# svenstaro/bvh

Measured on NVIDIA H100. Metric: traversal_Mrays_per_s, higher is better.
Workload: dtype f32

## Files before the change

bvh_b200/csrc/traverse.cu:

```cuda
#include "internal.h"
#include "csr.cuh"
#include "queries.cuh"
#include <cstdlib>
#include <cstring>
#include <algorithm>
#include <chrono>

namespace bvhb200 {

static inline uint32_t pick_slots(bvhgpu_ctx* ctx, uint32_t nrays) {
    if (ctx->traverse_slots >= 0) return (uint32_t)std::min<int64_t>(ctx->traverse_slots, 64);
    uint64_t budget_words = 1ull << 30;
    if (ctx->slot_budget_words == 0) {
        size_t free_b = 0, total_b = 0;
        ctx->slot_budget_words = cudaMemGetInfo(&free_b, &total_b) == cudaSuccess ? std::max<uint64_t>((uint64_t)free_b / 16, 1) : budget_words;
    }
    budget_words = std::min<uint64_t>(budget_words, ctx->slot_budget_words);
    const uint64_t k = budget_words / std::max<uint32_t>(nrays, 1u);
    if (k < 4) return (uint32_t)k;
    uint32_t p = 4;
    while (p * 2 <= k && p < 64) p *= 2;
    return p;
}

template <class T> static inline const typename Traits<T>::DAabb* walk_aabbs(const Tree<T>* tree) { return tree->dims == 2 && tree->d_aabb_trav ? tree->d_aabb_trav : tree->d_aabb; }

constexpr int SCAN_ITEMS = 8;
constexpr int SCAN_THREADS = 256;
constexpr int SCAN_TILE = SCAN_ITEMS * SCAN_THREADS;
static_assert(SCAN_THREADS == CSR_SCAN_THREADS && SCAN_TILE == CSR_SCAN_TILE, "scan geometry declared in internal.h");

template <class T> __device__ __forceinline__ T tmin2(T a, T b);
template <> __device__ __forceinline__ float tmin2(float a, float b) { return fminf(a, b); }
template <> __device__ __forceinline__ double tmin2(double a, double b) { return fmin(a, b); }
template <class T> __device__ __forceinline__ T tmax2(T a, T b);
template <> __device__ __forceinline__ float tmax2(float a, float b) { return fmaxf(a, b); }
template <> __device__ __forceinline__ double tmax2(double a, double b) { return fmax(a, b); }

template <class T>
__device__ __forceinline__ bool slab_hit(const T o[3], const T inv[3], const T mn[3], const T mx[3]) {
    const T l0 = mul_rn(sub_rn(mn[0], o[0]), inv[0]), r0 = mul_rn(sub_rn(mx[0], o[0]), inv[0]);
    const T l1 = mul_rn(sub_rn(mn[1], o[1]), inv[1]), r1 = mul_rn(sub_rn(mx[1], o[1]), inv[1]);
    const T l2 = mul_rn(sub_rn(mn[2], o[2]), inv[2]), r2 = mul_rn(sub_rn(mx[2], o[2]), inv[2]);
    const bool nan = (l0 != l0) | (r0 != r0) | (l1 != l1) | (r1 != r1) | (l2 != l2) | (r2 != r2);
    const T tmin = tmax2(tmax2(tmin2(l0, r0), tmin2(l1, r1)), tmin2(l2, r2));
    const T tmax = tmin2(tmin2(tmax2(l0, r0), tmax2(l1, r1)), tmax2(l2, r2));
    const T lo = tmin > T(0) ? tmin : T(0);
    return !nan && tmax >= lo;
}

template <class T, bool FLAT, class Emit>
__device__ __forceinline__ uint32_t walk(const typename Traits<T>::TNode* __restrict__ trec, uint32_t n_rec,
                                         const typename Traits<T>::DAabb* __restrict__ aabb,
                                         const T o[3], const T inv[3], Emit emit) {
    uint32_t i = 0, visits = 0;
    while (i < n_rec) {
        T mn[3], mx[3];
        uint32_t skip, shape;
        fetch(trec + i, mn, mx, skip, shape);
        ++visits;
        if (slab_hit(o, inv, mn, mx)) {
            if (shape != BVH_INVALID) {
                bool report = true;
                if (FLAT) {
                    T smn[3], smx[3];
                    load_aabb(aabb + shape, smn, smx);
                    report = slab_hit(o, inv, smn, smx);
                }
                if (report) emit(shape);
            }
            i = i + 1;
        } else {
            i = skip;
        }
    }
    return visits;
}

template <class T> struct RaySrc { const T* base; uint32_t fmt; };
constexpr uint32_t RAYS_FULL = 0, RAYS_OD = 1;
template <class T, bool L2>
__device__ __forceinline__ void load_ray(const RaySrc<T>& src, size_t r, T o[3], T inv[3]) {
    if (src.fmt == RAYS_FULL) {
        const T* p = src.base + 9 * r;
#pragma unroll
        for (int k = 0; k < 3; ++k) { o[k] = L2 ? __ldcg(p + k) : __ldg(p + k); inv[k] = L2 ? __ldcg(p + 6 + k) : __ldg(p + 6 + k); }
    } else {
        const T* p = src.base + 6 * r;
#pragma unroll
        for (int k = 0; k < 3; ++k) { o[k] = L2 ? __ldcg(p + k) : __ldg(p + k); inv[k] = div_rn(T(1), L2 ? __ldcg(p + 3 + k) : __ldg(p + 3 + k)); }
    }
}

template <class T>
__global__ void __launch_bounds__(256) coherence_probe_kernel(RaySrc<T> rays, uint32_t nrays, uint32_t* flag) {
    __shared__ float acc[8];
    float sum = 0.f;
    const uint32_t samples = 1024, stride = nrays > 2 * samples ? nrays / samples : 1;
    const uint32_t rstride = rays.fmt == RAYS_FULL ? 9u : 6u;
    uint32_t n = 0;
    for (uint32_t k = threadIdx.x; k < samples; k += 256) {
        const uint32_t i = k * stride;
        if (i + 1 >= nrays) break;
        const T* a = rays.base + (size_t)rstride * i + 3;
        const T* b = rays.base + (size_t)rstride * (i + 1) + 3;
        sum += (float)(a[0] * b[0] + a[1] * b[1] + a[2] * b[2]);
        ++n;
    }
    for (int o = 16; o > 0; o >>= 1) { sum += __shfl_xor_sync(0xffffffffu, sum, o); n += __shfl_xor_sync(0xffffffffu, n, o); }
    __shared__ uint32_t cnt[8];
    if (lane_id() == 0) { acc[threadIdx.x >> 5] = sum; cnt[threadIdx.x >> 5] = n; }
    __syncthreads();
    if (threadIdx.x == 0) {
        float s = 0.f; uint32_t c = 0;
        for (int w = 0; w < 8; ++w) { s += acc[w]; c += cnt[w]; }
        *flag = (c > 0 && s / (float)c > 0.9f) ? 1u : 0u;
    }
}

template <class T, bool FLAT>
__global__ void __launch_bounds__(256) walk_count_kernel(const typename Traits<T>::TNode* __restrict__ trec, uint32_t n_rec,
                                                         const typename Traits<T>::DAabb* __restrict__ aabb,
                                                         RaySrc<T> rays, uint32_t nrays,
                                                         uint32_t first, uint32_t count,
                                                         uint32_t* __restrict__ counts, uint32_t* __restrict__ slots, uint32_t K,
                                                         unsigned long long* __restrict__ visit_total, const uint32_t* __restrict__ gate, uint32_t run_if) {
    if (gate && *gate != run_if) return;
    const uint32_t r = first + blockIdx.x * blockDim.x + threadIdx.x;
    uint32_t visits = 0;
    if (r < first + count) {
        T o[3], inv[3];
        load_ray<T, false>(rays, r, o, inv);
        uint32_t cnt = 0;
        visits = walk<T, FLAT>(trec, n_rec, aabb, o, inv, [&](uint32_t shape) {
            if (cnt < K) slots[(size_t)cnt * nrays + r] = shape;
            ++cnt;
        });
        counts[r] = cnt;
    }
    visits = __reduce_add_sync(0xffffffffu, visits);
    if (lane_id() == 0 && visits) atomicAdd(visit_total, (unsigned long long)visits);
}

template <class T, bool FLAT, bool STREAM>
__global__ void __launch_bounds__(256) walk_persistent_kernel(const typename Traits<T>::TNode* __restrict__ trec, uint32_t n_rec,
                                                              const typename Traits<T>::DAabb* __restrict__ aabb,
                                                              RaySrc<T> rays, uint32_t nrays,
                                                              uint32_t* __restrict__ ticket, const uint32_t* ready,
                                                              uint32_t* __restrict__ counts, uint32_t* __restrict__ slots, uint32_t K,
                                                              unsigned long long* __restrict__ visit_total, const uint32_t* __restrict__ gate, uint32_t run_if,
                                                              uint32_t* err, unsigned long long timeout_ns) {
    if (gate && *gate != run_if) return;
    constexpr uint32_t NONE = 0xFFFFFFFFu;
    constexpr int REFILL = 8;
    const uint32_t FULL = 0xffffffffu;
    const uint32_t lane = lane_id(), lt = lanemask_lt();
    uint32_t r = NONE, i = 0, cnt = 0, visits = 0;
    bool loaded = false;
    T o[3] = {T(0), T(0), T(0)}, inv[3] = {T(0), T(0), T(0)};
    bool exhausted = false;
    for (;;) {
        const uint32_t need = __ballot_sync(FULL, r == NONE);
        if (need && !exhausted) {
            uint32_t base = 0;
            if (lane == 0) base = atomicAdd(ticket, (uint32_t)__popc(need));
            base = __shfl_sync(FULL, base, 0);
            if (base >= nrays) exhausted = true;
            const uint32_t mine = base + __popc(need & lt);
            if (r == NONE && mine < nrays) {
                r = mine; i = 0; cnt = 0;
                if (STREAM) loaded = false;
                else load_ray<T, false>(rays, mine, o, inv);
            }
        }
        if (STREAM) {
            const uint32_t pend = __ballot_sync(FULL, r != NONE && !loaded);
            if (pend) {
                const bool any_active = __ballot_sync(FULL, r != NONE && loaded) != 0u;
                const uint32_t lowest = __reduce_min_sync(FULL, (r != NONE && !loaded) ? r : NONE);
                uint32_t rd = 0, ok = 1;
                if (lane == 0) {
                    rd = *(volatile const uint32_t*)ready;
                    if (!any_active && rd <= lowest) {
                        uint32_t ns = 100;
                        const unsigned long long t0 = global_timer_ns();
                        while (rd <= lowest) {
                            if (*(volatile const uint32_t*)err != 0u) { ok = 0; break; }
                            if (global_timer_ns() - t0 > timeout_ns) { ok = 0; atomicExch(err, (uint32_t)BVHGPU_ERR_TIMEOUT); break; }
                            __nanosleep(ns);
                            if (ns < 2000) ns <<= 1;
                            rd = *(volatile const uint32_t*)ready;
                        }
                    }
                }
                rd = __shfl_sync(FULL, rd, 0);
                ok = __shfl_sync(FULL, ok, 0);
                if (!ok) {
                    exhausted = true;
                    if (r != NONE && !loaded) r = NONE;
                } else if (__ballot_sync(FULL, r != NONE && !loaded && r < rd)) {
                    __threadfence();
                    if (r != NONE && !loaded && r < rd) { load_ray<T, true>(rays, r, o, inv); loaded = true; }
                }
            }
        }
        if (__ballot_sync(FULL, r != NONE) == 0) break;
        uint32_t rounds = 0;
        for (;;) {
            if (r != NONE && (!STREAM || loaded)) {
                T mn[3], mx[3];
                uint32_t skip, shape;
                fetch(trec + i, mn, mx, skip, shape);
                ++visits;
                if (slab_hit(o, inv, mn, mx)) {
                    if (shape != BVH_INVALID) {
                        bool report = true;
                        if (FLAT) {
                            T smn[3], smx[3];
                            load_aabb(aabb + shape, smn, smx);
                            report = slab_hit(o, inv, smn, smx);
                        }
                        if (report) { if (cnt < K) slots[(size_t)cnt * nrays + r] = shape; ++cnt; }
                    }
                    i = i + 1;
                } else {
                    i = skip;
                }
                if (i >= n_rec) { counts[r] = cnt; r = NONE; }
            }
            const uint32_t idle_mask = __ballot_sync(FULL, r == NONE);
            const int idle = __popc(idle_mask);
            if (idle == 32 || (idle >= REFILL && !exhausted)) break;
            if (STREAM) {
                const uint32_t pend = __ballot_sync(FULL, r != NONE && !loaded);
                if (pend && (((++rounds) & 15u) == 0u || (pend | idle_mask) == FULL)) break;
            }
        }
    }
    visits = __reduce_add_sync(FULL, visits);
    if (lane == 0 && visits) atomicAdd(visit_total, (unsigned long long)visits);
}

template <bool FLAT, bool STREAM, int VPC>
__global__ void __launch_bounds__(1024, 1) walk_top_kernel(const TNodeF* __restrict__ trec, const DAabbF* __restrict__ aabb,
                                                           uint32_t n_rec, const float4* __restrict__ top,
                                                           RaySrc<float> rays, uint32_t nrays, uint32_t* __restrict__ ticket, const uint32_t* ready,
                                                           uint32_t* __restrict__ counts, uint32_t* __restrict__ slots, uint32_t K,
                                                           unsigned long long* __restrict__ visit_total, const uint32_t* __restrict__ gate, uint32_t run_if,
                                                           uint32_t* err, unsigned long long timeout_ns, int refill) {
    extern __shared__ float4 s_top[];
    if (gate && *gate != run_if) return;
    const uint32_t n_top = reinterpret_cast<const uint32_t*>(top)[0];
    for (uint32_t k = threadIdx.x; k < 2 * n_top; k += blockDim.x) s_top[k] = top[2 + k];
    __syncthreads();
    uint32_t s_lo;
    asm volatile("mov.u32 %0, %1;" : "=r"(s_lo) : "r"((uint32_t)__cvta_generic_to_shared(s_top)));
    const uint32_t s_hi = s_lo + 16u * n_top;
    constexpr uint32_t NONE = 0xFFFFFFFFu;
    const uint32_t FULL = 0xffffffffu;
    const uint32_t lane = lane_id(), lt = lanemask_lt();
    uint32_t r = NONE, j = 0, g = 0, gend = 0, cnt = 0, visits = 0;
    bool loaded = false;
    float o[3] = {0.f, 0.f, 0.f}, inv[3] = {0.f, 0.f, 0.f};
    bool exhausted = false;
    for (;;) {
        const uint32_t need = __ballot_sync(FULL, r == NONE);
        if (need && !exhausted) {
            uint32_t base = 0;
            if (lane == 0) base = atomicAdd(ticket, (uint32_t)__popc(need));
            base = __shfl_sync(FULL, base, 0);
            if (base >= nrays) exhausted = true;
            const uint32_t mine = base + __popc(need & lt);
            if (r == NONE && mine < nrays) {
                r = mine; j = 0; cnt = 0; g = 0; gend = n_top ? 0u : n_rec;
                if (STREAM) loaded = false;
                else load_ray<float, false>(rays, mine, o, inv);
            }
        }
        if (STREAM) {
            const uint32_t pend = __ballot_sync(FULL, r != NONE && !loaded);
            if (pend) {
                const bool any_active = __ballot_sync(FULL, r != NONE && loaded) != 0u;
                const uint32_t lowest = __reduce_min_sync(FULL, (r != NONE && !loaded) ? r : NONE);
                uint32_t rd = 0, ok = 1;
                if (lane == 0) {
                    rd = *(volatile const uint32_t*)ready;
                    if (!any_active && rd <= lowest) {
                        uint32_t ns = 100;
                        const unsigned long long t0 = global_timer_ns();
                        while (rd <= lowest) {
                            if (*(volatile const uint32_t*)err != 0u) { ok = 0; break; }
                            if (global_timer_ns() - t0 > timeout_ns) { ok = 0; atomicExch(err, (uint32_t)BVHGPU_ERR_TIMEOUT); break; }
                            __nanosleep(ns);
                            if (ns < 2000) ns <<= 1;
                            rd = *(volatile const uint32_t*)ready;
                        }
                    }
                }
                rd = __shfl_sync(FULL, rd, 0);
                ok = __shfl_sync(FULL, ok, 0);
                if (!ok) {
                    exhausted = true;
                    if (r != NONE && !loaded) r = NONE;
                } else if (__ballot_sync(FULL, r != NONE && !loaded && r < rd)) {
                    __threadfence();
                    if (r != NONE && !loaded && r < rd) { load_ray<float, true>(rays, r, o, inv); loaded = true; }
                }
            }
        }
        if (__ballot_sync(FULL, r != NONE) == 0) break;
        const int leave = exhausted ? 32 : refill;
        auto visit = [&]() {
            if (r != NONE && (!STREAM || loaded)) {
                float mn[3], mx[3];
                uint32_t w3, w7;
                const bool below = g < gend;
                if (!below) {
                    float4 a, b;
                    asm("ld.shared.v4.f32 {%0,%1,%2,%3}, [%4];" : "=f"(a.x), "=f"(a.y), "=f"(a.z), "=f"(a.w) : "r"(s_lo + 16u * j));
                    asm("ld.shared.v4.f32 {%0,%1,%2,%3}, [%4];" : "=f"(b.x), "=f"(b.y), "=f"(b.z), "=f"(b.w) : "r"(s_hi + 16u * j));
                    mn[0] = a.x; mn[1] = a.y; mn[2] = a.z; w3 = __float_as_uint(a.w);
                    mx[0] = b.x; mx[1] = b.y; mx[2] = b.z; w7 = __float_as_uint(b.w);
                } else {
                    fetch(trec + g, mn, mx, w3, w7);
                }
                ++visits;
                const bool hit = slab_hit(o, inv, mn, mx);
                const bool fringe = !below && (w7 + 0x80000000u) < 0x7FFFFFFFu;
                const uint32_t cur = below ? g : j;
                const uint32_t nxt = (hit || fringe) ? cur + 1 : w3;
                if (hit && (int32_t)w7 >= 0) {
                    bool report = true;
                    if (FLAT) {
                        float smn[3], smx[3];
                        load_aabb(aabb + w7, smn, smx);
                        report = slab_hit(o, inv, smn, smx);
                    }
                    if (report) { if (cnt < K) slots[(size_t)cnt * nrays + r] = w7; ++cnt; }
                }
                j = below ? j : nxt;
                gend = below ? gend : ((hit && fringe) ? w3 : 0u);
                g = below ? nxt : (w7 & 0x7FFFFFFFu);
                if (g >= gend && j >= n_top) { counts[r] = cnt; r = NONE; }
            }
        };
        uint32_t rounds = 0;
        for (;;) {
#pragma unroll
            for (int u = 0; u < VPC; ++u) visit();
            const uint32_t idle_mask = __ballot_sync(FULL, r == NONE);
            if (__popc(idle_mask) >= leave) break;
            if (STREAM) {
                const uint32_t pend = __ballot_sync(FULL, r != NONE && !loaded);
                if (pend && (((rounds += VPC) & 15u) == 0u || (pend | idle_mask) == FULL)) break;
            }
        }
    }
    visits = __reduce_add_sync(FULL, visits);
    if (lane == 0 && visits) atomicAdd(visit_total, (unsigned long long)visits);
}

__global__ void __launch_bounds__(SCAN_THREADS) scan_local_kernel(const uint32_t* __restrict__ counts, uint32_t n,
                                                                  uint32_t* __restrict__ local, unsigned long long* __restrict__ blocksum,
                                                                  uint32_t* __restrict__ maxcount) {
    __shared__ uint32_t wsum[SCAN_THREADS / 32];
    const uint32_t base = blockIdx.x * SCAN_TILE + threadIdx.x * SCAN_ITEMS;
    uint32_t v[SCAN_ITEMS], s = 0, m = 0;
#pragma unroll
    for (int k = 0; k < SCAN_ITEMS; ++k) { v[k] = (base + k < n) ? counts[base + k] : 0u; s += v[k]; m = v[k] > m ? v[k] : m; }
    uint32_t incl = s;
#pragma unroll
    for (int o = 1; o < 32; o <<= 1) { const uint32_t t = __shfl_up_sync(0xffffffffu, incl, o); if ((int)lane_id() >= o) incl += t; }
    if (lane_id() == 31) wsum[threadIdx.x >> 5] = incl;
    if (maxcount) { m = __reduce_max_sync(0xffffffffu, m); if (lane_id() == 0 && m) atomicMax(maxcount, m); }
    __syncthreads();
    uint32_t woff = 0;
    for (int w = 0; w < (int)(threadIdx.x >> 5); ++w) woff += wsum[w];
    uint32_t run = woff + incl - s;
#pragma unroll
    for (int k = 0; k < SCAN_ITEMS; ++k) { if (base + k < n) local[base + k] = run; run += v[k]; }
    if (threadIdx.x == SCAN_THREADS - 1) blocksum[blockIdx.x] = (unsigned long long)(woff + incl);
}
__global__ void __launch_bounds__(1024) scan_blocks_kernel(unsigned long long* __restrict__ blocksum, uint32_t nblocks,
                                                           unsigned long long* __restrict__ total) {
    __shared__ unsigned long long wsum[32];
    __shared__ unsigned long long carry_s;
    if (threadIdx.x == 0) carry_s = *total;
    __syncthreads();
    for (uint32_t b0 = 0; b0 < nblocks; b0 += 1024) {
        const uint32_t b = b0 + threadIdx.x;
        const unsigned long long v = b < nblocks ? blocksum[b] : 0ull;
        unsigned long long incl = v;
#pragma unroll
        for (int o = 1; o < 32; o <<= 1) { const unsigned long long t = __shfl_up_sync(0xffffffffu, incl, o); if ((int)lane_id() >= o) incl += t; }
        if (lane_id() == 31) wsum[threadIdx.x >> 5] = incl;
        __syncthreads();
        unsigned long long woff = 0;
        for (int w = 0; w < (int)(threadIdx.x >> 5); ++w) woff += wsum[w];
        const unsigned long long carry = carry_s;
        if (b < nblocks) blocksum[b] = carry + woff + incl - v;
        __syncthreads();
        if (threadIdx.x == 1023) carry_s = carry + woff + incl;
        __syncthreads();
    }
    if (threadIdx.x == 0) *total = carry_s;
}

__device__ __forceinline__ void st_release_sys(unsigned long long* p, unsigned long long v) {
    asm volatile("st.release.sys.global.u64 [%0], %1;" ::"l"(p), "l"(v) : "memory");
}
__device__ __forceinline__ unsigned long long ld_acquire_sys(const unsigned long long* p) {
    unsigned long long v;
    asm volatile("ld.acquire.sys.global.u64 %0, [%1];" : "=l"(v) : "l"(p) : "memory");
    return v;
}
constexpr int MB_TOT = 0, MB_DONE = 64, MB_TRACE = 128, MB_TRACE_LEN = 1024;
constexpr unsigned long long TILE_BYTES = 4ull * SCAN_TILE;
constexpr unsigned long long OFF_MASK = (1ull << 56) - 1ull;
struct PeerBoxes {
    int rank, world;
    unsigned long long* box[BVHGPU_MAX_PEERS];
    unsigned char* stage[BVHGPU_MAX_PEERS];
    uint32_t* hits[BVHGPU_MAX_PEERS];
    unsigned long long seq;
    unsigned long long rays_before[BVHGPU_MAX_PEERS + 1];
    unsigned long long tiles_before[BVHGPU_MAX_PEERS + 1];
    unsigned long long table_off;
    uint32_t* err;
    unsigned long long timeout_ns;
};

struct XInfo { unsigned long long base[BVHGPU_MAX_PEERS], grand, waited; };
__device__ __forceinline__ void wait_posts(const PeerBoxes& pb, XInfo* xs) {
    const int lane = threadIdx.x;
    const unsigned long long par = pb.seq & 1ull;
    unsigned long long tot = 0, waited = 0;
    if (lane < pb.world) {
        const unsigned long long* slot = pb.box[pb.rank] + MB_TOT + (par * BVHGPU_MAX_PEERS + lane) * 4;
        const unsigned long long t0 = global_timer_ns();
        uint32_t spins = 0;
        while (ld_acquire_sys(slot) != pb.seq) {
            if (((++spins) & 63u) == 0u && global_timer_ns() - t0 > pb.timeout_ns) { atomicExch(pb.err, (uint32_t)BVHGPU_ERR_TIMEOUT); break; }
            __nanosleep(100);
        }
        tot = slot[1];
        waited = global_timer_ns() - t0;
    }
    unsigned long long run = 0, wmax = 0, mine = 0;
    for (int r = 0; r < pb.world; ++r) {
        const unsigned long long v = __shfl_sync(0xffffffffu, tot, r), w = __shfl_sync(0xffffffffu, waited, r);
        if (lane == r) mine = run;
        run += v;
        wmax = w > wmax ? w : wmax;
    }
    if (lane < BVHGPU_MAX_PEERS) xs->base[lane] = mine;
    if (lane == 0) { xs->grand = run; xs->waited = wmax; }
}

template <bool SHARDED>
__global__ void __launch_bounds__(SCAN_THREADS) scan_post_kernel(const uint32_t* __restrict__ counts, uint32_t n, uint32_t* __restrict__ local,
                                                                 unsigned long long* __restrict__ blocksum, unsigned long long* __restrict__ total,
                                                                 uint32_t* __restrict__ arrival, PeerBoxes pb, unsigned long long* __restrict__ xinfo) {
    __shared__ uint32_t wsum[SCAN_THREADS / 32], wmax[SCAN_THREADS / 32];
    __shared__ XInfo xs;
    __shared__ unsigned long long wsum64[SCAN_THREADS / 32];
    __shared__ unsigned long long carry_s;
    __shared__ bool last;
    const uint32_t base = blockIdx.x * SCAN_TILE + threadIdx.x * SCAN_ITEMS;
    uint32_t v[SCAN_ITEMS], s = 0, m = 0;
#pragma unroll
    for (int k = 0; k < SCAN_ITEMS; ++k) { v[k] = (base + k < n) ? counts[base + k] : 0u; s += v[k]; m = v[k] > m ? v[k] : m; }
    uint32_t incl = s;
#pragma unroll
    for (int o = 1; o < 32; o <<= 1) { const uint32_t t = __shfl_up_sync(0xffffffffu, incl, o); if ((int)lane_id() >= o) incl += t; }
    m = __reduce_max_sync(0xffffffffu, m);
    if (lane_id() == 31) wsum[threadIdx.x >> 5] = incl;
    if (lane_id() == 0) wmax[threadIdx.x >> 5] = m;
    __syncthreads();
    uint32_t woff = 0, tsum = 0, tmax = 0;
#pragma unroll
    for (int w = 0; w < SCAN_THREADS / 32; ++w) { if (w < (int)(threadIdx.x >> 5)) woff += wsum[w]; tsum += wsum[w]; tmax = wmax[w] > tmax ? wmax[w] : tmax; }
    uint32_t run = woff + incl - s;
#pragma unroll
    for (int k = 0; k < SCAN_ITEMS; ++k) { if (base + k < n) local[base + k] = run; run += v[k]; }
    const unsigned long long width = tmax <= 0xFFu ? 1ull : (tmax <= 0xFFFFu ? 2ull : 4ull);
    if (SHARDED) {
        unsigned long long tb_mine = 0;
#pragma unroll
        for (int k = 1; k < BVHGPU_MAX_PEERS; ++k) if (k == pb.rank) tb_mine = pb.tiles_before[k];
        const unsigned long long at = TILE_BYTES * (tb_mine + blockIdx.x) + (unsigned long long)threadIdx.x * SCAN_ITEMS * width;
        if (width == 1) {
            const uint2 q = make_uint2(v[0] | v[1] << 8 | v[2] << 16 | v[3] << 24, v[4] | v[5] << 8 | v[6] << 16 | v[7] << 24);
#pragma unroll
            for (int d = 0; d < BVHGPU_MAX_PEERS; ++d) if (d < pb.world) *reinterpret_cast<uint2*>(pb.stage[d] + at) = q;
        } else if (width == 2) {
            const uint4 q = make_uint4(v[0] | v[1] << 16, v[2] | v[3] << 16, v[4] | v[5] << 16, v[6] | v[7] << 16);
#pragma unroll
            for (int d = 0; d < BVHGPU_MAX_PEERS; ++d) if (d < pb.world) *reinterpret_cast<uint4*>(pb.stage[d] + at) = q;
        } else {
            const uint4 q0 = make_uint4(v[0], v[1], v[2], v[3]), q1 = make_uint4(v[4], v[5], v[6], v[7]);
#pragma unroll
            for (int d = 0; d < BVHGPU_MAX_PEERS; ++d) if (d < pb.world) { *reinterpret_cast<uint4*>(pb.stage[d] + at) = q0; *reinterpret_cast<uint4*>(pb.stage[d] + at + 16) = q1; }
        }
    }
    if (threadIdx.x == 0) blocksum[blockIdx.x] = (unsigned long long)tsum | (width << 56);
    __syncthreads();
    if (threadIdx.x == 0) {
        if (SHARDED && pb.world > 1) __threadfence_system(); else __threadfence();
        last = atomicAdd(arrival, 1u) == gridDim.x - 1;
    }
    __syncthreads();
    if (!last) return;
    if (threadIdx.x == 0) { __threadfence(); carry_s = 0ull; }
    __syncthreads();
    unsigned long long tb_mine = 0;
    if (SHARDED) {
#pragma unroll
        for (int k = 1; k < BVHGPU_MAX_PEERS; ++k) if (k == pb.rank) tb_mine = pb.tiles_before[k];
    }
    for (uint32_t b0 = 0; b0 < gridDim.x; b0 += SCAN_THREADS) {
        const uint32_t bb = b0 + threadIdx.x;
        const unsigned long long e = bb < gridDim.x ? __ldcg(blocksum + bb) : 0ull;
        const unsigned long long val = e & OFF_MASK;
        unsigned long long in64 = val;
#pragma unroll
        for (int o = 1; o < 32; o <<= 1) { const unsigned long long t = __shfl_up_sync(0xffffffffu, in64, o); if ((int)lane_id() >= o) in64 += t; }
        if (lane_id() == 31) wsum64[threadIdx.x >> 5] = in64;
        __syncthreads();
        unsigned long long wo = 0;
        for (int w = 0; w < (int)(threadIdx.x >> 5); ++w) wo += wsum64[w];
        const unsigned long long carry = carry_s;
        const unsigned long long excl = carry + wo + in64 - val;
        if (bb < gridDim.x) {
            blocksum[bb] = excl;
            if (SHARDED) {
                const unsigned long long entry = (excl & OFF_MASK) | (e & ~OFF_MASK);
#pragma unroll
                for (int d = 0; d < BVHGPU_MAX_PEERS; ++d) if (d < pb.world) *reinterpret_cast<unsigned long long*>(pb.stage[d] + pb.table_off + 8ull * (tb_mine + bb)) = entry;
            }
        }
        __syncthreads();
        if (threadIdx.x == SCAN_THREADS - 1) carry_s = carry + wo + in64;
        __syncthreads();
    }
    if (threadIdx.x == 0) { *total = carry_s; *arrival = 0u; }
    if (SHARDED) {
        if (threadIdx.x == 0) __threadfence_system();
        __syncthreads();
        if (threadIdx.x < (unsigned)pb.world) {
            unsigned long long* slot = pb.box[threadIdx.x] + MB_TOT + ((pb.seq & 1ull) * BVHGPU_MAX_PEERS + pb.rank) * 4;
            slot[1] = carry_s;
            __threadfence_system();
            st_release_sys(slot, pb.seq);
        }
        __syncthreads();
        if (threadIdx.x < 32) {
            wait_posts(pb, &xs);
            __syncwarp();
            if (threadIdx.x < BVHGPU_MAX_PEERS) xinfo[threadIdx.x] = xs.base[threadIdx.x];
            if (threadIdx.x == 0) { xinfo[8] = xs.grand; xinfo[9] = xs.waited; }
        }
    }
}

__device__ __forceinline__ void goffsets_body(const PeerBoxes& pb, const unsigned long long* __restrict__ xinfo, uint32_t* __restrict__ offsets,
                                              uint32_t bid, uint32_t ntiles) {
    __shared__ uint32_t wsum[SCAN_THREADS / 32];
    __shared__ uint32_t failed;
    if (threadIdx.x == 0) failed = *(volatile uint32_t*)pb.err;
    __syncthreads();
    const unsigned long long g = bid;
    if (failed == 0u) {
        int sg = 0;
        unsigned long long tb = 0, rb = 0, re = pb.rays_before[1];
#pragma unroll
        for (int k = 1; k < BVHGPU_MAX_PEERS; ++k) if (k < pb.world && g >= pb.tiles_before[k]) { sg = k; tb = pb.tiles_before[k]; rb = pb.rays_before[k]; re = pb.rays_before[k + 1]; }
        const unsigned long long hb = xinfo[sg];
        const unsigned char* stage = nullptr;
#pragma unroll
        for (int d = 0; d < BVHGPU_MAX_PEERS; ++d) if (d == pb.rank) stage = pb.stage[d];
        const unsigned long long entry = __ldcg(reinterpret_cast<const unsigned long long*>(stage + pb.table_off + 8ull * g));
        const unsigned long long width = entry >> 56;
        const unsigned char* p = stage + TILE_BYTES * g + (unsigned long long)threadIdx.x * SCAN_ITEMS * width;
        uint32_t v[SCAN_ITEMS], s = 0;
        static_assert(SCAN_ITEMS == 8, "8 counts per thread");
        if (width == 1) {
            const uint2 q = __ldcg(reinterpret_cast<const uint2*>(p));
            v[0] = q.x & 0xFFu; v[1] = (q.x >> 8) & 0xFFu; v[2] = (q.x >> 16) & 0xFFu; v[3] = q.x >> 24; v[4] = q.y & 0xFFu; v[5] = (q.y >> 8) & 0xFFu; v[6] = (q.y >> 16) & 0xFFu; v[7] = q.y >> 24;
        } else if (width == 2) {
            const uint4 q = __ldcg(reinterpret_cast<const uint4*>(p));
            v[0] = q.x & 0xFFFFu; v[1] = q.x >> 16; v[2] = q.y & 0xFFFFu; v[3] = q.y >> 16; v[4] = q.z & 0xFFFFu; v[5] = q.z >> 16; v[6] = q.w & 0xFFFFu; v[7] = q.w >> 16;
        } else {
            const uint4 q0 = __ldcg(reinterpret_cast<const uint4*>(p)), q1 = __ldcg(reinterpret_cast<const uint4*>(p) + 1);
            v[0] = q0.x; v[1] = q0.y; v[2] = q0.z; v[3] = q0.w; v[4] = q1.x; v[5] = q1.y; v[6] = q1.z; v[7] = q1.w;
        }
#pragma unroll
        for (int k = 0; k < SCAN_ITEMS; ++k) s += v[k];
        uint32_t incl = s;
#pragma unroll
        for (int o = 1; o < 32; o <<= 1) { const uint32_t t = __shfl_up_sync(0xffffffffu, incl, o); if ((int)lane_id() >= o) incl += t; }
        if (lane_id() == 31) wsum[threadIdx.x >> 5] = incl;
        __syncthreads();
        uint32_t woff = 0;
        for (int w = 0; w < (int)(threadIdx.x >> 5); ++w) woff += wsum[w];
        unsigned long long run = hb + (entry & OFF_MASK) + woff + incl - s;
        const unsigned long long j0 = rb + (g - tb) * SCAN_TILE + (unsigned long long)threadIdx.x * SCAN_ITEMS;
        uint32_t ov[SCAN_ITEMS];
#pragma unroll
        for (int k = 0; k < SCAN_ITEMS; ++k) { ov[k] = run > 0xFFFFFFFFull ? 0xFFFFFFFFu : (uint32_t)run; run += v[k]; }
        if (j0 + SCAN_ITEMS <= re && (j0 & 3ull) == 0ull) {
            uint4* o4 = reinterpret_cast<uint4*>(offsets + j0);
            o4[0] = make_uint4(ov[0], ov[1], ov[2], ov[3]);
            o4[1] = make_uint4(ov[4], ov[5], ov[6], ov[7]);
        } else {
#pragma unroll
            for (int k = 0; k < SCAN_ITEMS; ++k) if (j0 + k < re) offsets[j0 + k] = ov[k];
        }
        if (g == ntiles - 1 && threadIdx.x == 0) {
            unsigned long long ng = 0;
#pragma unroll
            for (int k = 1; k <= BVHGPU_MAX_PEERS; ++k) if (k == pb.world) ng = pb.rays_before[k];
            const unsigned long long grand = xinfo[8];
            offsets[ng] = grand > 0xFFFFFFFFull ? 0xFFFFFFFFu : (uint32_t)grand;
        }
    }
    if (bid == 0 && threadIdx.x < 32) {
        const int lane = threadIdx.x;
        const unsigned long long par = pb.seq & 1ull;
        unsigned long long waited = 0;
        if (lane < pb.world) {
            const unsigned long long* slot = pb.box[pb.rank] + MB_DONE + par * BVHGPU_MAX_PEERS + lane;
            const unsigned long long t0 = global_timer_ns();
            uint32_t spins = 0;
            while (ld_acquire_sys(slot) != pb.seq) {
                if (((++spins) & 63u) == 0u && global_timer_ns() - t0 > pb.timeout_ns) { atomicExch(pb.err, (uint32_t)BVHGPU_ERR_TIMEOUT); break; }
                __nanosleep(100);
            }
            waited = global_timer_ns() - t0;
        }
        for (int o = 16; o > 0; o >>= 1) { const unsigned long long w = __shfl_xor_sync(0xffffffffu, waited, o); waited = w > waited ? w : waited; }
        if (lane == 0) {
            unsigned long long* tr = pb.box[pb.rank] + MB_TRACE + (pb.seq % MB_TRACE_LEN) * 4;
            tr[0] = pb.seq; tr[1] = global_timer_ns(); tr[2] = xinfo[9]; tr[3] = waited;
        }
    }
}

struct EmitDst {
    uint32_t* offsets;
    uint32_t* hits;
    unsigned long long nrays_out;
};
// ... 798 lines not shown
```

Baseline: 2434.

## Predicate top-level BVH node fetches and use NaN-propagating min/max in slab test

Adds a float specialization of the slab test that uses min.NaN/max.NaN PTX, so the six explicit NaN comparisons are no longer needed. For VPC>1 it swaps the branchy visit for a branch-free one: predicated shared/global vector loads, conditional index updates, and a ray-completion check once per VPC batch rather than per visit. Traversal state is now initialized when the ray is loaded, so an unloaded ray never walks. The aim is to cut warp divergence and instruction count in the inner loop, at the cost of idle or finished lanes doing wasted predicated work and rays retiring late, up to VPC-1 visits after they finish.

```diff
diff --git a/bvh_b200/csrc/traverse.cu b/bvh_b200/csrc/traverse.cu
--- a/bvh_b200/csrc/traverse.cu
+++ b/bvh_b200/csrc/traverse.cu
@@ -47,6 +47,18 @@
     const T tmax = tmin2(tmin2(tmax2(l0, r0), tmax2(l1, r1)), tmax2(l2, r2));
     const T lo = tmin > T(0) ? tmin : T(0);
     return !nan && tmax >= lo;
+}
+__device__ __forceinline__ float fmin_nan(float a, float b) { float r; asm("min.NaN.f32 %0, %1, %2;" : "=f"(r) : "f"(a), "f"(b)); return r; }
+__device__ __forceinline__ float fmax_nan(float a, float b) { float r; asm("max.NaN.f32 %0, %1, %2;" : "=f"(r) : "f"(a), "f"(b)); return r; }
+template <>
+__device__ __forceinline__ bool slab_hit<float>(const float o[3], const float inv[3], const float mn[3], const float mx[3]) {
+    const float l0 = mul_rn(sub_rn(mn[0], o[0]), inv[0]), r0 = mul_rn(sub_rn(mx[0], o[0]), inv[0]);
+    const float l1 = mul_rn(sub_rn(mn[1], o[1]), inv[1]), r1 = mul_rn(sub_rn(mx[1], o[1]), inv[1]);
+    const float l2 = mul_rn(sub_rn(mn[2], o[2]), inv[2]), r2 = mul_rn(sub_rn(mx[2], o[2]), inv[2]);
+    const float tmin = fmax_nan(fmax_nan(fmin_nan(l0, r0), fmin_nan(l1, r1)), fmin_nan(l2, r2));
+    const float tmax = fmin_nan(fmin_nan(fmax_nan(l0, r0), fmax_nan(l1, r1)), fmax_nan(l2, r2));
+    const float lo = tmin > 0.f ? tmin : 0.f;
+    return tmax >= lo;
 }
 
 template <class T, bool FLAT, class Emit>
@@ -253,15 +265,16 @@
     const uint32_t n_top = reinterpret_cast<const uint32_t*>(top)[0];
     for (uint32_t k = threadIdx.x; k < 2 * n_top; k += blockDim.x) s_top[k] = top[2 + k];
     __syncthreads();
-    uint32_t s_lo;
+    uint32_t s_lo, s_hi;
     asm volatile("mov.u32 %0, %1;" : "=r"(s_lo) : "r"((uint32_t)__cvta_generic_to_shared(s_top)));
-    const uint32_t s_hi = s_lo + 16u * n_top;
+    asm volatile("mov.u32 %0, %1;" : "=r"(s_hi) : "r"(s_lo + 16u * n_top));
     constexpr uint32_t NONE = 0xFFFFFFFFu;
     const uint32_t FULL = 0xffffffffu;
     const uint32_t lane = lane_id(), lt = lanemask_lt();
-    uint32_t r = NONE, j = 0, g = 0, gend = 0, cnt = 0, visits = 0;
+    uint32_t r = NONE, j = NONE, g = 0, gend = 0, cnt = 0, visits = 0;
     bool loaded = false;
     float o[3] = {0.f, 0.f, 0.f}, inv[3] = {0.f, 0.f, 0.f};
+    float4 a = make_float4(0.f, 0.f, 0.f, 0.f), b = a;
     bool exhausted = false;
     for (;;) {
         const uint32_t need = __ballot_sync(FULL, r == NONE);
@@ -272,9 +285,9 @@
             if (base >= nrays) exhausted = true;
             const uint32_t mine = base + __popc(need & lt);
             if (r == NONE && mine < nrays) {
-                r = mine; j = 0; cnt = 0; g = 0; gend = n_top ? 0u : n_rec;
-                if (STREAM) loaded = false;
-                else load_ray<float, false>(rays, mine, o, inv);
+                r = mine; cnt = 0; g = 0;
+                if (STREAM) { loaded = false; j = NONE; gend = 0; }
+                else { j = 0; gend = n_top ? 0u : n_rec; load_ray<float, false>(rays, mine, o, inv); }
             }
         }
         if (STREAM) {
@@ -304,23 +317,26 @@
                     if (r != NONE && !loaded) r = NONE;
                 } else if (__ballot_sync(FULL, r != NONE && !loaded && r < rd)) {
                     __threadfence();
-                    if (r != NONE && !loaded && r < rd) { load_ray<float, true>(rays, r, o, inv); loaded = true; }
+                    if (r != NONE && !loaded && r < rd) {
+                        load_ray<float, true>(rays, r, o, inv); loaded = true;
+                        j = 0; gend = n_top ? 0u : n_rec;
+                    }
                 }
             }
         }
         if (__ballot_sync(FULL, r != NONE) == 0) break;
         const int leave = exhausted ? 32 : refill;
-        auto visit = [&]() {
+        auto visit_branchy = [&]() {
             if (r != NONE && (!STREAM || loaded)) {
                 float mn[3], mx[3];
                 uint32_t w3, w7;
                 const bool below = g < gend;
                 if (!below) {
-                    float4 a, b;
-                    asm("ld.shared.v4.f32 {%0,%1,%2,%3}, [%4];" : "=f"(a.x), "=f"(a.y), "=f"(a.z), "=f"(a.w) : "r"(s_lo + 16u * j));
-                    asm("ld.shared.v4.f32 {%0,%1,%2,%3}, [%4];" : "=f"(b.x), "=f"(b.y), "=f"(b.z), "=f"(b.w) : "r"(s_hi + 16u * j));
-                    mn[0] = a.x; mn[1] = a.y; mn[2] = a.z; w3 = __float_as_uint(a.w);
-                    mx[0] = b.x; mx[1] = b.y; mx[2] = b.z; w7 = __float_as_uint(b.w);
+                    float4 lo4, hi4;
+                    asm("ld.shared.v4.f32 {%0,%1,%2,%3}, [%4];" : "=f"(lo4.x), "=f"(lo4.y), "=f"(lo4.z), "=f"(lo4.w) : "r"(s_lo + 16u * j));
+                    asm("ld.shared.v4.f32 {%0,%1,%2,%3}, [%4];" : "=f"(hi4.x), "=f"(hi4.y), "=f"(hi4.z), "=f"(hi4.w) : "r"(s_hi + 16u * j));
+                    mn[0] = lo4.x; mn[1] = lo4.y; mn[2] = lo4.z; w3 = __float_as_uint(lo4.w);
+                    mx[0] = hi4.x; mx[1] = hi4.y; mx[2] = hi4.z; w7 = __float_as_uint(hi4.w);
                 } else {
                     fetch(trec + g, mn, mx, w3, w7);
                 }
@@ -344,10 +360,47 @@
                 if (g >= gend && j >= n_top) { counts[r] = cnt; r = NONE; }
             }
         };
+        auto visit = [&]() {
+            const bool below = g < gend;
+            const bool top = !below && j < n_top;
+            const bool walking = below || top;
+            const TNodeF* gp = trec + g;
+            asm("{\n\t.reg .pred pt, pb;\n\t"
+                "setp.ne.u32 pt, %10, 0;\n\tsetp.ne.u32 pb, %11, 0;\n\t"
+                "@pt ld.shared.v4.f32 {%0,%1,%2,%3}, [%8];\n\t"
+                "@pt ld.shared.v4.f32 {%4,%5,%6,%7}, [%9];\n\t"
+                "@pb ld.global.nc.v4.f32 {%0,%1,%2,%3}, [%12];\n\t"
+                "@pb ld.global.nc.v4.f32 {%4,%5,%6,%7}, [%12+16];\n\t}"
+                : "+f"(a.x), "+f"(a.y), "+f"(a.z), "+f"(a.w), "+f"(b.x), "+f"(b.y), "+f"(b.z), "+f"(b.w)
+                : "r"(s_lo + 16u * j), "r"(s_hi + 16u * j), "r"((uint32_t)top), "r"((uint32_t)below), "l"(gp));
+            const float mn[3] = {a.x, a.y, a.z}, mx[3] = {b.x, b.y, b.z};
+            const uint32_t w3 = __float_as_uint(a.w), w7 = __float_as_uint(b.w);
+            visits += walking;
+            const bool hit = walking & slab_hit(o, inv, mn, mx);
+            const bool fringe = (int32_t)w7 < -1;
+            const bool adv = hit || fringe;
+            if (hit && (int32_t)w7 >= 0) {
+                bool report = true;
+                if (FLAT) {
+                    float smn[3], smx[3];
+                    load_aabb(aabb + w7, smn, smx);
+                    report = slab_hit(o, inv, smn, smx);
+                }
+                if (report) { if (cnt < K) slots[(size_t)cnt * nrays + r] = w7; ++cnt; }
+            }
+            if (top) j = adv ? j + 1 : w3;
+            if (below) g = adv ? g + 1 : w3;
+            if (hit && fringe) { g = w7 & 0x7FFFFFFFu; gend = w3; }
+        };
         uint32_t rounds = 0;
         for (;;) {
-#pragma unroll
-            for (int u = 0; u < VPC; ++u) visit();
+            if constexpr (VPC == 1) {
+                visit_branchy();
+            } else {
+#pragma unroll
+                for (int u = 0; u < VPC; ++u) visit();
+                if (r != NONE && (!STREAM || loaded) && g >= gend && j >= n_top) { counts[r] = cnt; r = NONE; }
+            }
             const uint32_t idle_mask = __ballot_sync(FULL, r == NONE);
             if (__popc(idle_mask) >= leave) break;
             if (STREAM) {
```

After: 2682, median of 6. +10.2%, better.
